# jgrodzki/radix_sort

Measured on AMD Instinct MI355X. Metric: Gkeys/sec (u64), higher is better.
Workload: dtype u64

## Files before the change

radix_sort_amd/csrc/rsx.hip:

```cpp
#include "rsx_internal.hpp"
#include "rsx_misc_kernels.hpp"
#include "rsx_any_kernels.hpp"

#include <cmath>

using namespace rsx;
using namespace rsxh;

namespace {

bool layout_ok(const rsx_layout* L, bool any_width = false) {
    if (!L) return false;
    const uint32_t kb = L->key_bytes;
    if (any_width ? (kb < 1 || kb > 16) : !(kb == 1 || kb == 2 || kb == 4 || kb == 8 || kb == 16)) return false;
    if (L->key_kind > RSX_KEY_FLOAT) return false;
    if (L->key_kind == RSX_KEY_FLOAT && !(kb == 4 || kb == 8)) return false;
    if (L->elem_bytes == 0 || (uint64_t)L->key_offset + kb > L->elem_bytes) return false;
    return true;
}
const EsLaunchers* launchers_for(uint32_t es) {
    switch (es) {
        case 1: return &es_launchers<1>();
        case 2: return &es_launchers<2>();
        case 4: return &es_launchers<4>();
// ... 247 lines not shown
                       BT, xor_mask);
    RSX_HIP(hipGetLastError());
    ctx->last_path = PATH_COUNT16;
    return RSX_OK;
}

uint32_t wide_cap(uint32_t es) { return bucket_cape((int)es, wide_kpt_for((int)es), 1024); }
bool wide_forecast(rsx_ctx* ctx, size_t n, const rsx_layout* L, hipStream_t st) {
    const uint32_t es = L->elem_bytes, D = L->key_bytes;
    const bool wide_type = es >= 8 && D >= 4;
    const size_t wide_floor = D >= 8 ? 0 : es == 8 ? ((size_t)1 << 30) : ((size_t)2 << 30);
    const bool wide_size = wide_type && (uint64_t)n > mid_max_elems((int)es);
    bool wide = false;
    if (ctx->wide_mode == 2) {
        wide = wide_type && n >= 65536;
    } else if (((ctx->wide_mode == 1 && n * (size_t)es >= wide_floor) || ctx->wide_mode == 3) && wide_size &&
               (uint64_t)n / 65536u < (uint64_t)wide_cap(es)) {
        volatile uint32_t& hint = host_word(ctx, HV_WIDE_HINT);
        const uint64_t sig = 1ull | (uint64_t)(63 - __builtin_clzll((unsigned long long)n)) << 8 | (uint64_t)es << 16 | (uint64_t)L->key_offset << 24 |
                             (uint64_t)D << 32 | (uint64_t)L->key_kind << 40;
        if (ctx->wide_skip > 0 && sig == ctx->wide_refused_sig) {
            --ctx->wide_skip;
        } else if (hint == 2u && sig == ctx->wide_tried_sig) {
            hint = 0;
            ctx->wide_skip = 15;
            ctx->wide_refused_sig = sig;
        } else {
            if (hint == 2u) hint = 0;
            wide = true;
            ctx->wide_tried_sig = sig;
        }
    }
    return wide && !((ctx->ovf16 == nullptr || ctx->wide_buf == nullptr) && capturing(st));
}
int sort_wide(rsx_ctx* ctx, const EsLaunchers& K, void* d_data, void* d_tmp, size_t n, const rsx_layout* L, hipStream_t st) {
    const uint32_t es = L->elem_bytes, D = L->key_bytes;
    int rc = ensure_ovf16(ctx, st);
    if (rc) return rc;
    if (!ctx->wide_buf) {
        RSX_HIP(hipMalloc(reinterpret_cast<void**>(&ctx->wide_buf), WIDE_BUF_BYTES));
        RSX_HIP(hipMemsetAsync(reinterpret_cast<char*>(ctx->wide_buf) + WIDE_PLAN_OFFSET, 0, sizeof(WidePlan), st));
    }
    uint64_t* tot = reinterpret_cast<uint64_t*>(ctx->wide_buf);
    uint64_t* BT = tot + 65536;
    uint64_t* starts = BT + 256;
    WidePlan* plan = reinterpret_cast<WidePlan*>(reinterpret_cast<char*>(ctx->wide_buf) + WIDE_PLAN_OFFSET);
    const uint32_t* verdict = &plan->verdict;
    const RegionGeom geom = make_geom(ctx, n, es);
    size_t parts = n * (size_t)es / (32768 * sizeof(uint32_t));
    if (parts > (size_t)ctx->num_cu) parts = (size_t)ctx->num_cu;
    static_assert(bucket_cape(8, wide_kpt_for(8), 1024) < 0x8000u && bucket_cape(4, wide_kpt_for(4), 1024) < 0x8000u, "a bucket that fits LDS must not overflow a 16-bit counter");
    uint32_t k = ctx->wide_mode == 2 ? 0u : (uint32_t)(parts / geom.num_regions);
    if (k > 0) parts = (size_t)k * geom.num_regions;
    rc = K.wideplan(ctx, d_data, n, L, plan, st);
    if (rc) return rc;
    rc = K.count16top(ctx, d_data, n, L, plan, static_cast<uint32_t*>(d_tmp), (uint32_t)parts, geom.region_shift, k, st);
    if (rc) return rc;
    {
        LaunchTimer lt(ctx, RSX_PROF_SCAN, st);
        hipLaunchKernelGGL(rsx_total16_kernel, dim3(256), dim3(256), 0, st, static_cast<const uint32_t*>(d_tmp), (uint32_t)parts, ctx->ovf16, tot, BT);
        RSX_HIP(hipGetLastError());
        const uint64_t cap1024 = wide_big_form((int)es, n) ? wide_cap(es) : bucket_cap((int)es), cap512 = bucket_cap((int)es) / 2;
        hipLaunchKernelGGL(rsx_scan16_kernel, dim3(256), dim3(256), 0, st, tot, BT, starts, cap512 / 2, cap512, cap1024, group_shift(ctx, n, L),
                           ctx->wide_mode == 2 ? 1u : 0u, (uint64_t)bucket_cape((int)es, medium_kpt_for((int)es), 1024) * 150u, (uint64_t)n / 64u, plan,
                           ctx->host_err_dev + HV_WIDE_HINT, reinterpret_cast<uint32_t*>(ctx->wide_buf + WIDE_LEFT_OFFSET));
        RSX_HIP(hipGetLastError());
    }
    SortRun lsd;
    rc = begin_control(ctx, lsd, st, geom, false);
    if (rc) return rc;
    ctx->cb_last = lsd.cb;
    SortRun hyb = lsd;
    hyb.gate = Gate{verdict, VERDICT_PATH_MASK, VERDICT_HYBRID};
    hyb.spec_dev = &plan->specs[0];
    if (k > 0) {
        rc = K.marginal16(ctx, hyb, static_cast<const uint32_t*>(d_tmp), (uint32_t)parts, k, geom, J_of(ctx, hyb, 0), J_of(ctx, hyb, 1), st);
    } else {
        rc = K.hist(ctx, hyb, d_data, geom, L, D - 2, J_of(ctx, hyb, 0), J_of(ctx, hyb, 1), true, st);
    }
    if (rc) return rc;
    rc = K.sweep(ctx, hyb, SweepPass{0, false, 0}, d_data, d_tmp, geom, L, D - 2, J_of(ctx, hyb, 0), J_of(ctx, hyb, 1), nullptr, 1, st);
    if (rc) return rc;
    hyb.spec_dev = &plan->specs[1];
    rc = K.sweep(ctx, hyb, SweepPass{1, true, 0}, d_tmp, d_data, geom, L, D - 1, J_of(ctx, hyb, 1), nullptr, nullptr, 0, st);
    if (rc) return rc;
    rc = K.bucket16(ctx, hyb, d_data, d_tmp, n, L, starts, plan, st);
    if (rc) return rc;
    lsd.gate = Gate{verdict, VERDICT_PATH_MASK, VERDICT_LSD};
    rc = lsd_passes(ctx, K, lsd, d_data, d_tmp, n, L, geom, false, 0, st);
    if (rc) return rc;
    ctx->last_sort_passes = D;
    ctx->last_path = PATH_WIDE;
    end_control(ctx);
    return RSX_OK;
}

uint32_t mid_forecast(rsx_ctx* ctx, size_t n, bool* bucket_small) {
    const uint32_t hint = host_word(ctx, HV_MID_HINT);
    uint32_t mid_mode;
    if (ctx->mid_choice == 1 && hint == 2 && ctx->mid_cooldown == 0) ctx->mid_cooldown = 8;
    if (ctx->mid_cooldown > 0) {
        --ctx->mid_cooldown;
        mid_mode = 2;
    } else {
        mid_mode = hint == 2 ? 2u : 1u;
    }
    if (ctx->mid_force) mid_mode = ctx->mid_force;
    ctx->mid_choice = mid_mode;
    *bucket_small = hint == 1 && (uint64_t)n <= 256ull * 2048ull;
    return mid_mode;
}
int sort_mid_split(rsx_ctx* ctx, const EsLaunchers& K, void* d_data, void* d_tmp, size_t n, const rsx_layout* L, bool bucket_small, hipStream_t st) {
    int rc = K.mid_split(ctx, d_data, d_tmp, n, L, st);
    if (rc) return rc;
    rc = K.bucket_sort(ctx, d_tmp, d_data, L, bucket_small, st);
    if (rc) return rc;
    ctx->last_path = PATH_MID_SPLIT;
    return RSX_OK;
}

int sort_lsd(rsx_ctx* ctx, const EsLaunchers& K, void* d_data, void* d_tmp, size_t n, const rsx_layout* L, bool mid, uint32_t mid_mode,
             hipStream_t st) {
    const RegionGeom geom = make_geom(ctx, n, L->elem_bytes);
    SortRun run;
    int rc = begin_control(ctx, run, st, geom, mid);
    if (rc) return rc;
    rc = lsd_passes(ctx, K, run, d_data, d_tmp, n, L, geom, mid, mid_mode, st);
    if (rc) return rc;
    end_control(ctx);
    return RSX_OK;
}

int sort_counting8(rsx_ctx* ctx, const EsLaunchers& K, void* d_data, size_t n, const rsx_layout* L, hipStream_t st) {
    const RegionGeom geom = make_geom(ctx, n, L->elem_bytes);
    SortRun run;
    int rc = begin_control(ctx, run, st, geom, false);
    if (rc) return rc;
    rc = K.hist(ctx, run, d_data, geom, L, 0, J_of(ctx, run, 0), nullptr, false, st);
    if (rc) return rc;
    LaunchTimer lt(ctx, RSX_PROF_OTHER, st);
    const uint64_t steps = ((n + 15) / 16 + 255) / 256;
    uint64_t blocks = steps;
    if (blocks > (uint64_t)ctx->num_cu * 16) blocks = (uint64_t)ctx->num_cu * 16;
    hipLaunchKernelGGL(rsx_expand_bytes_kernel, dim3((uint32_t)blocks), dim3(256), 0, st, static_cast<uint8_t*>(d_data),
                       (uint64_t)n, J_of(ctx, run, 0), geom.num_regions, status32(geom) ? 1u : 0u,
                       L->key_kind == RSX_KEY_SIGNED ? 0x80u : 0u);
    RSX_HIP(hipGetLastError());
    end_control(ctx);
    ctx->last_path = PATH_COUNT8;
    return RSX_OK;
}

int sort_device_locked(rsx_ctx* ctx, void* d_data, void* d_tmp, size_t n, const rsx_layout* L, hipStream_t st) {
    const EsLaunchers* K = launchers_for(L->elem_bytes);
    if (!K) return fail(ctx, RSX_ERR_UNSUPPORTED, "element size has no device kernel");
    int rc = pending_error(ctx);
    if (rc) return rc;
    rc = ensure_workspace(ctx, n, L, st);
    if (rc) return rc;
    Enqueue enq(ctx, st);
    const uint32_t D = L->key_bytes;
    const bool general_bytes = (ctx->options & OPT_GENERAL_BYTES) != 0;
    const bool counting8 = L->elem_bytes == 1 && !general_bytes;
    note_path(ctx, PATH_LSD, 0);
    if (!counting8 && n <= (size_t)512 * kpt_for((int)L->elem_bytes) && !(ctx->options & OPT_NO_SMALL_SORT)) {
        ctx->last_path = PATH_SMALL;
        return K->small_sort(ctx, d_data, n, L, st);
// ... 2427 lines not shown
```

radix_sort_amd/csrc/rsx_device.hpp:

```cpp
#pragma once
#include <hip/hip_runtime.h>
#include <stdint.h>

#include <type_traits>

namespace rsx {

constexpr int WAVE = 64;
constexpr int RADIX = 256;

template <int ES>
struct Elem;
template <>
struct Elem<1> {
    uint8_t w[1];
};
template <>
struct Elem<2> {
    uint16_t w[1];
};
template <>
struct alignas(4) Elem<4> {
    uint32_t w[1];
};
// ... 353 lines not shown
    static constexpr int SHIFT = 30;
    static constexpr uint32_t MASK = (1u << 30) - 1;
};
template <>
struct Status<uint64_t> {
    static constexpr int SHIFT = 62;
    static constexpr uint64_t MASK = (1ull << 62) - 1;
};

struct SweepArgs {
    const void* src;
    void* dst;
    RegionGeom g;
    const unsigned long long* J;
    void* status;
    uint32_t* tickets;
    const uint32_t* prev_mode;
    uint16_t wg_first[MAX_REGIONS + 1];
    void* status_clean;
    uint32_t rank_atomic;
    uint32_t hot_lanes;
    uint32_t tiles_per_region;
    uint32_t local_mask;
    unsigned long long* jnext;
    unsigned long long* jzero;
    uint32_t* error;
    DigitSpec spec;
    DigitSpec next;
    const DigitSpec* spec_dev;
    KeyXform xf;
    uint32_t opts;
    const unsigned long long* mid_J;
    DigitSpec mid_spec;
    uint32_t mid_cap;
    uint32_t mid_mode;
    uint32_t* mid_hint;
    Gate gate;
    uint32_t dbg;
    unsigned long long* dbg_cnt;
};
constexpr bool sweep_wide_cnt(int es, int kpt, int wg) { return es <= 4 && kpt >= 16 && wg <= 512; }
constexpr uint32_t SWEEP_OPT_DYNAMIC = 1u;
constexpr uint32_t SWEEP_OPT_NO_XCD_MAJOR = 2u;
constexpr uint32_t SWEEP_OPT_AGENT_STATUS = 4u;
constexpr uint32_t SWEEP_OPT_RANK_CHECK = 8u;
constexpr uint32_t SWEEP_OPT_PREREAD = 16u;
#ifdef RSX_TUNING
#define RSX_DBG(a, bit) ((a).dbg & (bit))
#else
#define RSX_DBG(a, bit) 0u
#endif

#ifdef RSX_STAMPS
#define RSX_STAMP(k)                                                   \
    do {                                                               \
        const unsigned long long _t = __builtin_amdgcn_s_memtime();    \
        stamp_acc[k] += _t - stamp_prev;                               \
        stamp_prev = _t;                                               \
    } while (0)
#else
#define RSX_STAMP(k) do {} while (0)
#endif
#ifndef RSX_MINW
#define RSX_MINW 6
#endif
#ifndef RSX_WO_PREREAD
#define RSX_WO_PREREAD 16
#endif
#ifndef RSX_START_STAGGER
#define RSX_START_STAGGER 224
#endif
#ifndef RSX_NUM_SGPR
#define RSX_NUM_SGPR 102
#endif
#ifndef RSX_RANK_GROUP
#define RSX_RANK_GROUP 4
#endif
#ifndef RSX_MINW_BIG
#define RSX_MINW_BIG 4
#endif
#ifndef RSX_WO_GROUP
#define RSX_WO_GROUP 4
#endif
#ifndef RSX_MINW_1024
#define RSX_MINW_1024 8
#endif
#ifndef RSX_ROLLCALL_TICKS
#define RSX_ROLLCALL_TICKS 40000
#endif

template <int ES, int KPT>
__device__ __forceinline__ void forget(Elem<ES> (&e)[KPT]) {
#pragma unroll
    for (int j = 0; j < KPT; ++j) {
        if constexpr (ES < 4) {
            uint32_t t = e[j].w[0];
            asm volatile("" : "+v"(t));
            e[j].w[0] = (decltype(e[j].w[0]))t;
        } else {
#pragma unroll
            for (int k = 0; k < ES / 4; ++k) asm volatile("" : "+v"(e[j].w[k]));
        }
    }
}

template <bool DPP>
__device__ __forceinline__ uint32_t wave_incl_scan(uint32_t x) {
  if constexpr (DPP) {
    auto step = [](uint32_t v, auto ctrl, auto rows) {
        return v + (uint32_t)__builtin_amdgcn_update_dpp(0, (int)v, decltype(ctrl)::value, decltype(rows)::value, 0xf, false);
    };
    x = step(x, std::integral_constant<int, 0x111>{}, std::integral_constant<int, 0xf>{});
    x = step(x, std::integral_constant<int, 0x112>{}, std::integral_constant<int, 0xf>{});
    x = step(x, std::integral_constant<int, 0x114>{}, std::integral_constant<int, 0xf>{});
    x = step(x, std::integral_constant<int, 0x118>{}, std::integral_constant<int, 0xf>{});
    x = step(x, std::integral_constant<int, 0x142>{}, std::integral_constant<int, 0xa>{});
    x = step(x, std::integral_constant<int, 0x143>{}, std::integral_constant<int, 0xc>{});
    return x;
  } else {
    const uint32_t lane = threadIdx.x & 63;
#pragma unroll
    for (int o = 1; o < 64; o <<= 1) {
        const uint32_t y = __shfl_up(x, o);
        if (lane >= (uint32_t)o) x += y;
    }
    return x;
  }
}

__device__ __forceinline__ void count_next(uint32_t* s_jn, uint32_t bin) {
    const uint32_t b0 = (uint32_t)__builtin_amdgcn_readfirstlane((int)bin);
    const uint64_t same = __ballot(bin == b0);
    if (bin == b0) {
        if (mbcnt64(same) == 0) atomicAdd(&s_jn[b0], (uint32_t)__popcll(same));
    } else {
        atomicAdd(&s_jn[bin], 1u);
    }
}

template <int ES, int KPT>
__device__ __forceinline__ void load_tile(Elem<ES> (&e)[KPT], const Elem<ES>* __restrict__ tile_ptr, uint32_t seg,
                                          uint32_t valid, bool full) {
    if (full) {
        const Elem<ES>* p0 = tile_ptr + seg;
#pragma unroll
        for (int j = 0; j < KPT; ++j) e[j] = p0[j * WAVE];
    } else {
#pragma unroll
        for (int j = 0; j < KPT; ++j) {
            const uint32_t p = seg + j * WAVE;
            if (p < valid) e[j] = tile_ptr[p];
            else e[j] = Elem<ES>{};
        }
    }
}

template <int ES, int KPT, int WG, typename S, int XF, bool NEXT, bool MID = false, bool STR = false>
__global__ __launch_bounds__(WG, (WG == 1024 ? RSX_MINW_1024 : ES == 16 ? 6 : KPT * (ES < 4 ? 4 : ES) >= 64 ? RSX_MINW_BIG : RSX_MINW))
__attribute__((amdgpu_num_sgpr(RSX_NUM_SGPR))) void rsx_sweep_kernel(const SweepArgs a) {
    constexpr int NWAVE = WG / WAVE;
    constexpr int TILE = WG * KPT;
    constexpr bool PREFETCH = ES >= 12;
    constexpr bool EARLY_HOP = ES <= 4;
    static_assert(WG >= RADIX, "need one thread per digit");
    static_assert(TILE <= 65536 / 2, "wave counters are 16 bit");
    using E = Elem<ES>;

    extern __shared__ __attribute__((aligned(16))) unsigned char smem[];
    constexpr size_t TILE_BYTES = (size_t)TILE * sizeof(E);
    E* s_elems = reinterpret_cast<E*>(smem);
    constexpr bool WIDE_CNT = sweep_wide_cnt(ES, KPT, WG);
    using Cnt = typename std::conditional<WIDE_CNT, uint32_t, uint16_t>::type;
    uint32_t* s_whist2 = reinterpret_cast<uint32_t*>(smem + TILE_BYTES);
    Cnt* s_whist = reinterpret_cast<Cnt*>(s_whist2);
    uint64_t* s_base = reinterpret_cast<uint64_t*>(s_whist2);
    uint32_t* s_jn = s_whist2 + NWAVE * RADIX * sizeof(Cnt) / 4;
    uint32_t* s_misc = s_jn + (NEXT ? a.g.num_regions * RADIX : 0);
    static_assert(NWAVE * RADIX * sizeof(Cnt) >= RADIX * sizeof(uint64_t), "s_base must fit in s_whist");

    if (!gate_open(a.gate)) return;
    const E* __restrict__ src = static_cast<const E*>(a.src);
    S* status = static_cast<S*>(a.status);
    const uint32_t NR = a.g.num_regions;
    const uint32_t tpr = a.tiles_per_region;
    const uint64_t region_len = 1ull << a.g.region_shift;

    if (NEXT)
        for (uint32_t i = threadIdx.x; i < a.g.num_regions * RADIX; i += WG) s_jn[i] = 0;
    using JT = S;
    if (a.jzero != nullptr)
        for (uint32_t i = blockIdx.x * WG + threadIdx.x; i < (uint32_t)J_REPL * NR * RADIX; i += gridDim.x * WG)
            reinterpret_cast<JT*>(a.jzero)[i] = 0;

    const uint32_t bx = (gridDim.x % 8u == 0u && !(a.opts & SWEEP_OPT_NO_XCD_MAJOR)) ? (blockIdx.x % 8u) * (gridDim.x / 8u) + blockIdx.x / 8u : blockIdx.x;
    uint32_t home = 0;
    while (home + 1 < NR && bx >= a.wg_first[home + 1]) ++home;
    const uint32_t st_step = a.wg_first[home + 1] - a.wg_first[home];
    uint32_t st_k = bx - a.wg_first[home];
    uint32_t st_nt;
    {
        const uint64_t rbeg = (uint64_t)home << a.g.region_shift;
        const uint64_t rlen = (a.g.n - rbeg) < region_len ? (a.g.n - rbeg) : region_len;
        st_nt = (uint32_t)((rlen + TILE - 1) / TILE);
    }
    E e[KPT];
    bool preloaded = false;
    uint64_t rbase = 0;
    uint64_t* s_scan = reinterpret_cast<uint64_t*>(s_misc + 16);
    uint64_t* s_half = reinterpret_cast<uint64_t*>(s_elems);
    static_assert(TILE_BYTES >= 2 * RADIX * sizeof(uint64_t), "scratch of the prefix phase lives in the tile area");
    auto load_counts = [&](const unsigned long long* Jm, uint32_t r, uint64_t& tot, uint64_t& below) {
        tot = 0;
        below = 0;
        constexpr uint32_t HALVES = WG >= 2 * RADIX ? 2 : 1;
        constexpr uint32_t RPH = J_REPL / HALVES;
        uint32_t t = threadIdx.x;
        asm volatile("" : "+v"(t));
        if (t < HALVES * RADIX) {
            const JT* col = reinterpret_cast<const JT*>(Jm) + (size_t)(t >> 8) * RPH * NR * RADIX + (t & 255u);
            constexpr uint32_t QU = ES >= 16 ? 4 : 8;
            for (uint32_t q0 = 0; q0 < NR; q0 += QU) {
#pragma unroll
                for (uint32_t qq = 0; qq < QU; ++qq) {
                    const uint32_t q = q0 + qq;
                    if (q < NR) {
#pragma unroll
                        for (uint32_t rep = 0; rep < RPH; ++rep) {
                            const uint64_t c = col[(size_t)(rep * NR + q) * RADIX];
                            tot += c;
                            below += q < r ? c : 0ull;
                        }
                    }
                }
            }
        }
    };
    auto scan_cursors = [&](uint64_t tot, uint64_t below) {
        const uint32_t t = threadIdx.x;
        if (WG >= 2 * RADIX && t >= RADIX && t < 2 * RADIX) {
            s_half[t - RADIX] = tot;
            s_half[t] = below;
        }
        __syncthreads();
        if (WG >= 2 * RADIX && t < RADIX) {
            tot += s_half[t];
            below += s_half[RADIX + t];
// ... 443 lines not shown
            }
            uint32_t spins = 0;
#ifdef RSX_STAMPS
            const unsigned long long lbs_t0 = __builtin_amdgcn_s_memtime();
            if (tid == 0 && kt > 0) ++lbs_tiles;
#endif
            while (lb_left != 0) {
#ifdef RSX_STAMPS
                if (tid == 0) ++lbs_hops;
#endif
                if (!lb_step()) {
#ifdef RSX_STAMPS
                    if (tid == 0) ++lbs_spins;
#endif
                    if (++spins > (1u << 22)) {
                        __hip_atomic_store(a.error, 1u, __ATOMIC_RELAXED, __HIP_MEMORY_SCOPE_SYSTEM);
                        break;
                    }
                    __builtin_amdgcn_s_sleep(1);
                }
            }
#ifdef RSX_STAMPS
            if (tid == 0 && kt > 0) lbs_cycles += __builtin_amdgcn_s_memtime() - lbs_t0;
#endif
            s_base[tid] = rbase + (uint64_t)lb_excl - (uint64_t)tstart;
        }
        __syncthreads();
        RSX_STAMP(5);
        if (prefetch) issue_next();

        if (!RSX_DBG(a, 2u)) {
            E* __restrict__ dst = static_cast<E*>(a.dst);
            auto next_bin = [&](uint64_t idx, const E& x) -> uint32_t {
                uint32_t r;
                if constexpr (sizeof(S) == 4)
                    r = __builtin_amdgcn_alignbit((uint32_t)(idx >> 32), (uint32_t)idx, a.g.region_shift);
                else
                    r = (uint32_t)(idx >> a.g.region_shift);
                return (r << 8) | sweep_digit<ES, STR>(x, next);
            };
            if (full) {
                auto write_full = [&](auto crowd, uint32_t hot_nd) __attribute__((always_inline)) {
                    constexpr bool CROWD = decltype(crowd)::value;
                    uint32_t hot_bin = ~0u, hot_acc = 0;
                    auto hot_flush = [&]() __attribute__((always_inline)) {
                        if (hot_acc != 0 && lane == 0) atomicAdd(&s_jn[hot_bin], hot_acc);
                        hot_acc = 0;
                    };
#pragma unroll
                    for (int i = 0; i < KPT; ++i) {
                        const uint32_t p = i * WG + tid;
                        E x;
                        if (i < PREREAD && preread) x = e[i];
                        else x = s_elems[slot_of(i)];
                        const uint64_t idx = s_base[sweep_digit<ES, STR>(x, spec)] + p;
                        if constexpr ((XF & 2) != 0) {
                            E y = x;
                            key_map<ES, true>(y, a.xf);
                            dst[idx] = y;
                        } else {
                            dst[idx] = x;
                        }
                        if constexpr (NEXT) {
                          if (!MID || do_next) {
                            if constexpr (CROWD) {
                                const uint32_t bin = next_bin(idx, x);
                                uint64_t same = __ballot(bin == hot_bin);
                                if (same == 0) {
                                    hot_flush();
                                    hot_bin = ((uint32_t)__builtin_amdgcn_readfirstlane((int)(bin >> 8)) << 8) | hot_nd;
                                    same = __ballot(bin == hot_bin);
                                    if (same == 0) {
                                        hot_bin = (uint32_t)__builtin_amdgcn_readfirstlane((int)bin);
                                        same = __ballot(bin == hot_bin);
                                    }
                                }
                                hot_acc += (uint32_t)__popcll(same);
                                if (bin != hot_bin) atomicAdd(&s_jn[bin], 1u);
                            } else if (!RSX_DBG(a, 0x8u)) {
                                atomicAdd(&s_jn[next_bin(idx, x)], 1u);
                            }
                          }
                        }
                        if (i % RSX_WO_GROUP == RSX_WO_GROUP - 1) __builtin_amdgcn_sched_barrier(0);
                    }
                    if constexpr (NEXT && CROWD) hot_flush();
                };
                bool crowded_next = false;
                uint32_t hot_nd = 0;
                if (do_next) {
                    const uint32_t nd = sweep_digit<ES, STR>(s_elems[sw0], next);
                    hot_nd = (uint32_t)__builtin_amdgcn_readfirstlane((int)nd);
                    crowded_next = __popcll(__ballot(nd == hot_nd)) >= 16;
                }
                if (crowded_next) write_full(std::true_type{}, hot_nd);
                else write_full(std::false_type{}, 0u);
            } else {
#pragma unroll
                for (int i = 0; i < KPT; ++i) {
                    const uint32_t p = i * WG + tid;
                    if (p < valid) {
                        const E x = s_elems[slot_of(i)];
                        const uint64_t idx = s_base[sweep_digit<ES, STR>(x, spec)] + p;
                        if constexpr ((XF & 2) != 0) {
                            E y = x;
                            key_map<ES, true>(y, a.xf);
                            dst[idx] = y;
                        } else {
                            dst[idx] = x;
                        }
                        if (do_next)
                            count_next(s_jn, next_bin(idx, x));
                    }
                }
            }
        }
        __syncthreads();
        RSX_STAMP(6);
    }

    if (do_next) {
        for (uint32_t i = threadIdx.x; i < a.g.num_regions * RADIX; i += WG) {
            const uint32_t c = s_jn[i];
            if (c)
                __hip_atomic_fetch_add(reinterpret_cast<JT*>(a.jnext) + (blockIdx.x % J_REPL) * (a.g.num_regions * RADIX) + i, (JT)c,
                                       __ATOMIC_RELAXED, __HIP_MEMORY_SCOPE_AGENT);
        }
    }
#ifdef RSX_STAMPS
    asm volatile("s_waitcnt vmcnt(0)" ::: "memory");
    __syncthreads();
    const unsigned long long stamp_end = __builtin_amdgcn_s_memtime();
    if ((threadIdx.x & 63) == 0)
        for (int k = 0; k < 8; ++k) atomicAdd(&a.dbg_cnt[(threadIdx.x >> 6) * 8 + k], stamp_acc[k]);
    if (threadIdx.x == 0) {
        atomicAdd(&a.dbg_cnt[64], stamp_called - stamp_entry);
        atomicAdd(&a.dbg_cnt[65], stamp_loop - stamp_called);
        atomicAdd(&a.dbg_cnt[66], stamp_end - stamp_prev);
        atomicAdd(&a.dbg_cnt[67], 1ull);
        atomicAdd(&a.dbg_cnt[68], lbs_hops);
        atomicAdd(&a.dbg_cnt[69], lbs_spins);
        atomicAdd(&a.dbg_cnt[70], lbs_cycles);
        atomicAdd(&a.dbg_cnt[71], lbs_tiles);
    }
#endif
}

template <int ES>
__global__ __launch_bounds__(256) void rsx_segcopy_kernel(const Elem<ES>* __restrict__ src,
                                                          Elem<ES>* __restrict__ dst,
                                                          const uint64_t* __restrict__ src_off,
                                                          const uint64_t* __restrict__ dst_off,
                                                          const uint64_t* __restrict__ len, uint32_t nseg,
                                                          uint32_t blocks_per_seg) {
    const uint32_t seg = blockIdx.x / blocks_per_seg;
    const uint32_t sub = blockIdx.x % blocks_per_seg;
    if (seg >= nseg) return;
    const uint64_t L = len[seg];
    const uint64_t so = src_off[seg], dof = dst_off[seg];
    for (uint64_t i = (uint64_t)sub * blockDim.x + threadIdx.x; i < L; i += (uint64_t)blocks_per_seg * blockDim.x)
        dst[dof + i] = src[so + i];
}

enum : uint32_t {
    SEGP_VALUES = 0,
    SEGP_LOCAL = 1,
// ... 5 lines not shown
```

radix_sort_amd/csrc/rsx_internal.hpp:

```cpp
#pragma once
#include "rsx_device.hpp"

#include <hip/hip_runtime.h>

#include <cstdio>
#include <cstdlib>
#include <cstring>
#include <mutex>
#include <new>
#include <algorithm>
#include <string>
#include <thread>
#include <utility>
#include <vector>

#include "../../include/rsx.h"

namespace rsxh {
using namespace rsx;

constexpr int MAX_PASSES = 16;
constexpr size_t J_BYTES = (size_t)J_REPL * MAX_REGIONS * RADIX * sizeof(uint64_t);
constexpr size_t TICKET_WORDS = ROLL_SHARDS + (size_t)ROLL_SHARD_COUNT * ROLL_SHARD_STRIDE;
constexpr uint32_t PART_MAX_SUB = 16;
// ... 143 lines not shown
        hipError_t _e = (call);                                         \
        if (_e != hipSuccess) return fail(ctx, RSX_ERR_HIP, #call, _e); \
    } while (0)

struct LaunchTimer {
    rsx_ctx* c;
    int kind;
    hipStream_t st;
    std::pair<hipEvent_t, hipEvent_t> ev{nullptr, nullptr};
    LaunchTimer(rsx_ctx* ctx, int k, hipStream_t s) : c(ctx), kind(k), st(s) {
        if (!c->prof) return;
        if (!c->prof_free.empty()) {
            ev = c->prof_free.back();
            c->prof_free.pop_back();
        } else if (hipEventCreate(&ev.first) != hipSuccess || hipEventCreate(&ev.second) != hipSuccess) {
            ev = {nullptr, nullptr};
            return;
        }
        (void)hipEventRecord(ev.first, st);
    }
    ~LaunchTimer() {
        if (!ev.first) return;
        (void)hipEventRecord(ev.second, st);
        c->prof_pending[kind].push_back(ev);
    }
};

#ifndef RSX_REGION_FLOOR
#define RSX_REGION_FLOOR 6
#endif
#ifndef RSX_KPT4
#define RSX_KPT4 28
#endif
#ifndef RSX_KPT2
#define RSX_KPT2 RSX_KPT4
#endif
#ifndef RSX_WG4
#define RSX_WG4 512
#endif
#ifndef RSX_KPT8
#define RSX_KPT8 14
#endif
#ifndef RSX_KPT16
#define RSX_KPT16 5
#endif
#ifndef RSX_KPT12
#define RSX_KPT12 10
#endif
#ifndef RSX_KPT32
#define RSX_KPT32 3
#endif
#ifndef RSX_KPT24
#define RSX_KPT24 5
#endif
#ifndef RSX_WG8
#define RSX_WG8 512
#endif
constexpr int bucket_kpt_for(int es) { return es <= 4 ? 28 : es == 8 ? 17 : es == 12 ? 9 : es == 16 ? 7 : es == 24 ? 4 : 3; }
constexpr int wide_kpt_for(int es) { return es <= 4 ? 28 : es == 8 ? 17 : es == 12 ? 12 : es == 16 ? 9 : es == 24 ? 6 : 5; }
#ifndef RSX_KMED8
#define RSX_KMED8 15
#endif
constexpr int medium_kpt_for(int es) { return es == 8 ? RSX_KMED8 : wide_kpt_for(es); }
constexpr bool wide_big_form(int es, uint64_t n) { return n / 65536u > (uint64_t)1024 * (uint64_t)bucket_kpt_for(es) * 7u / 8u; }
constexpr uint32_t LDS_PER_CU = 163840u;
constexpr size_t bucket_cnt_bytes() { return 4; }
constexpr uint32_t lds_tile_fixed(int wg) { return (uint32_t)(wg / 64) * 256u * (uint32_t)bucket_cnt_bytes() + 64u + 3u * 256u * 4u; }
constexpr uint32_t bucket_cape(int es, int kpt, int wg) {
    const uint32_t slots = (uint32_t)wg * (uint32_t)kpt;
    const uint32_t room = ((LDS_PER_CU - 1024u - lds_tile_fixed(wg)) / (uint32_t)es) & ~3u;
    return slots < room ? slots : room;
}
constexpr size_t lds_tile_bytes(int es, int kpt, int wg) { return (size_t)bucket_cape(es, kpt, wg) * (size_t)es + lds_tile_fixed(wg); }
constexpr uint32_t segment_cap(int es, int cls) { return bucket_cape(es, bucket_kpt_for(es), cls == 0 ? 256 : 1024); }
constexpr size_t WIDE_PLAN_OFFSET = (65536 + 256 + 65537 + 1) * sizeof(uint64_t);
constexpr size_t WIDE_LEFT_OFFSET = (WIDE_PLAN_OFFSET + sizeof(WidePlan) + 127) / 128 * 128;
constexpr size_t WIDE_DONE_OFFSET = WIDE_LEFT_OFFSET + 128;
constexpr size_t WIDE_BUF_BYTES = WIDE_DONE_OFFSET + 65536;
constexpr uint32_t bucket_cap(int es) { return 1024u * (uint32_t)bucket_kpt_for(es); }
constexpr uint64_t mid_max_elems(int es) { return es == 1 ? 0 : es == 8 ? (1ull << 22) : (uint64_t)bucket_cap(es) * 256u * 4u / 7u; }
constexpr int kpt_for(int es) { return es <= 2 ? RSX_KPT2 : es <= 4 ? RSX_KPT4 : es == 8 ? RSX_KPT8 : es == 12 ? RSX_KPT12 : es == 16 ? RSX_KPT16 : es == 24 ? RSX_KPT24 : RSX_KPT32; }
constexpr int wg_for(int es) { return es <= 4 ? RSX_WG4 : es == 8 ? RSX_WG8 : 512; }
constexpr uint32_t tile_elems(int es) { return wg_for(es) * kpt_for(es); }
constexpr int mid_kpt_for(int es) { return es <= 4 ? 8 : es == 8 ? 4 : es == 12 ? 3 : 2; }
constexpr uint32_t mid_tile_elems(int es) { return 512u * (uint32_t)mid_kpt_for(es); }

inline uint32_t log2u(uint64_t x) { return 63u - (uint32_t)__builtin_clzll(x); }

inline RegionGeom make_geom(const rsx_ctx* ctx, uint64_t n, uint32_t es, bool small_tiles = false) {
    RegionGeom g;
    g.n = n;
    g.tile = small_tiles ? mid_tile_elems((int)es) : tile_elems((int)es);
    uint32_t k = log2u(g.tile);
    if ((1ull << k) < g.tile) ++k;
    k += small_tiles ? 3 : RSX_REGION_FLOOR;
    const uint64_t cap = small_tiles ? MID_MAX_REGIONS : ctx->max_regions ? ctx->max_regions : (es == 8 || es == 32) ? 16 : 8;
    while (((n + (1ull << k) - 1) >> k) > cap) ++k;
    g.region_shift = k;
    g.num_regions = (uint32_t)((n + (1ull << k) - 1) >> k);
    if (g.num_regions == 0) g.num_regions = 1;
    return g;
}
inline uint64_t tiles_per_region(const RegionGeom& g) {
    return ((1ull << g.region_shift) + g.tile - 1) / g.tile;
}
inline uint64_t status_rows(const RegionGeom& g) {
    return (uint64_t)g.num_regions * tiles_per_region(g);
}
inline bool status32(const RegionGeom& g) { return g.region_shift <= 30; }

inline void ensure_lds(rsx_ctx* ctx, const void* kernel, size_t bytes) {
    for (const void* k : ctx->lds_attr)
        if (k == kernel) return;
    (void)hipFuncSetAttribute(kernel, hipFuncAttributeMaxDynamicSharedMemorySize, (int)bytes);
    ctx->lds_attr.push_back(kernel);
}

inline DigitSpec make_spec(const rsx_layout* L, uint32_t digit) {
    DigitSpec s;
    const uint32_t byte = L->key_offset + digit;
    const uint32_t top = L->key_offset + L->key_bytes - 1;
    if (L->elem_bytes >= 4) {
        s.word = byte >> 2;
        s.shift = 8 * (byte & 3);
        s.top_word = top >> 2;
        s.top_shift = 8 * (top & 3) + 7;
    } else {
        s.word = 0;
        s.shift = 8 * byte;
        s.top_word = 0;
        s.top_shift = 8 * top + 7;
    }
    s.flip = (L->key_kind != RSX_KEY_UNSIGNED && digit == L->key_bytes - 1) ? 0x80u : 0u;
    s.fsign = L->key_kind == RSX_KEY_FLOAT ? ~0u : 0u;
    return s;
}

inline char* cb_of(rsx_ctx* c, uint32_t which) { return c->aux + (size_t)which * CB_BYTES; }
inline unsigned long long* J_of(rsx_ctx* c, const SortRun& run, uint32_t which) {
    char* p = which == 0 ? cb_of(c, run.cb) + CB_J0 : which == 1 ? c->aux + OFF_J1 : c->aux + OFF_J2;
    return reinterpret_cast<unsigned long long*>(p);
}
inline unsigned long long* JT_of(rsx_ctx* c, const SortRun& run) { return reinterpret_cast<unsigned long long*>(cb_of(c, run.cb) + CB_JT); }
inline uint32_t* tickets_of(rsx_ctx* c, const SortRun& run, uint32_t pass) {
    return reinterpret_cast<uint32_t*>(cb_of(c, run.cb) + CB_TICKETS) + (size_t)pass * TICKET_WORDS;
}
inline uint32_t* part_tickets_of(rsx_ctx* c) { return reinterpret_cast<uint32_t*>(c->aux + OFF_PART_TICKETS); }
inline uint32_t* flags_of(rsx_ctx* c) { return reinterpret_cast<uint32_t*>(c->aux + OFF_FLAGS); }
inline volatile uint32_t& host_word(rsx_ctx* c, uint32_t w) { return reinterpret_cast<volatile uint32_t*>(c->host_err)[w]; }

inline uint32_t group_shift(const rsx_ctx* ctx, size_t n, const rsx_layout* L) {
    const uint64_t avg = (uint64_t)n / 65536u;
    uint32_t gs = 0;
    if (L->key_bytes >= 8 && ctx->bucket_group)
        while (gs < 6 && (avg << (gs + 1)) <= (uint64_t)512 * bucket_kpt_for((int)L->elem_bytes) * 3 / 4) ++gs;
    return gs >= 2 ? gs : 0;
}

struct SegPairsCall {
    void* keys;
    void* values;
    void* w0;
    void* w1;
    size_t n;
    uint32_t kb, vb;
    uint32_t kind, desc;
    uint32_t mode;
    uint32_t ib;
    const uint64_t* offsets;
    uint64_t nseg, row_len, max_len;
};
inline bool segment_pairs_mem(uint32_t es, const uint64_t* offsets, uint64_t row_len, uint64_t max_len) {
    const uint64_t cap = segment_cap((int)es, 1);
    return offsets ? (max_len == 0 || max_len > cap) : row_len > cap;
}

struct TopkCall {
    const void* keys;
    void* out_keys;
    void* out_index;
    void* w0;
    void* w1;
    uint64_t rows, row_len, k;
    uint32_t kb, kind, desc, ib;
};
inline uint32_t topk_max_k(uint32_t es) { return segment_cap((int)es, 1) / 2u; }
inline size_t topk_workspace_half(uint32_t es, uint64_t rows, uint64_t row_len, uint64_t k) {
    const uint64_t L = segment_cap((int)es, 1);
    if (row_len <= L) return 0;
    const uint64_t cpr = (row_len + L - 1) / L, last = row_len - (cpr - 1) * L;
// ... 157 lines not shown
```

radix_sort_amd/csrc/rsx_launch_impl.hpp:

```cpp
#pragma once
#include <cstdlib>
#include "rsx_internal.hpp"
#include "rsx_small_kernel.hpp"
#include "rsx_mid_kernels.hpp"
#include "rsx_segment_kernels.hpp"
#include "rsx_segment_pairs_kernels.hpp"
#include "rsx_topk_kernels.hpp"

#ifndef RSX_HIST_BLOCKS_PER_CU
#define RSX_HIST_BLOCKS_PER_CU 8
#endif

namespace rsxh {

inline uint32_t rank_atomic_of(const rsx_ctx* ctx) { return (ctx->rank_atomic && !(ctx->options & OPT_BALLOT_RANKS)) ? 1u : 0u; }
constexpr CleanList CLEAN_NONE = {{nullptr, nullptr, nullptr}, {0, 0, 0}};

inline uint64_t hist_blocks_per_region(const rsx_ctx* ctx, const RegionGeom& g) {
    const uint64_t per_block = 512ull * 16;
    uint64_t bpr = ((1ull << g.region_shift) + per_block - 1) / per_block;
    const uint64_t cap = ((uint64_t)ctx->num_cu * RSX_HIST_BLOCKS_PER_CU + g.num_regions - 1) / g.num_regions;
    if (bpr > cap) bpr = cap;
    return bpr == 0 ? 1 : bpr;
}
template <int ES, bool FLT>
int launch_hist_t(rsx_ctx* ctx, SortRun& run, const void* src, const RegionGeom& g, const rsx_layout* L, uint32_t digit,
                  unsigned long long* J, unsigned long long* jclear, bool clear_status, hipStream_t st) {
    const uint64_t zero16_n = clear_status ? status_rows(g) * RADIX * (status32(g) ? 4u : 8u) / 16u : 0u;
    const uint64_t bpr = hist_blocks_per_region(ctx, g);
    LaunchTimer lt(ctx, RSX_PROF_HIST, st);
    hipLaunchKernelGGL((rsx_hist_kernel<ES, FLT>), dim3((uint32_t)(bpr * g.num_regions)), dim3(512), 0, st,
                       static_cast<const Elem<ES>*>(src), g, make_spec(L, digit), (uint32_t)bpr, J, jclear, status32(g) ? 1u : 0u,
                       static_cast<uint4*>(ctx->status), zero16_n, run.clean, run.gate, DigitSpec{}, nullptr, run.spec_dev);
    RSX_HIP(hipGetLastError());
    run.clean = CLEAN_NONE;
    return RSX_OK;
}
template <int ES>
int launch_hist(rsx_ctx* ctx, SortRun& run, const void* src, const RegionGeom& g, const rsx_layout* L, uint32_t digit,
                unsigned long long* J, unsigned long long* jclear, bool clear_status, hipStream_t st) {
    if (L->key_kind == RSX_KEY_FLOAT || (L->key_kind == RSX_KEY_SIGNED && (digit + 1 == L->key_bytes || run.spec_dev != nullptr)))
        return launch_hist_t<ES, true>(ctx, run, src, g, L, digit, J, jclear, clear_status, st);
    return launch_hist_t<ES, false>(ctx, run, src, g, L, digit, J, jclear, clear_status, st);
}

template <int ES>
int launch_hist2(rsx_ctx* ctx, SortRun& run, const void* src, const RegionGeom& g, const rsx_layout* L, uint32_t digit,
                 unsigned long long* J, uint32_t digit2, unsigned long long* J2, unsigned long long* jclear, hipStream_t st) {
    const uint64_t zero16_n = status_rows(g) * RADIX * (status32(g) ? 4u : 8u) / 16u;
    const uint64_t bpr = hist_blocks_per_region(ctx, g);
    LaunchTimer lt(ctx, RSX_PROF_HIST, st);
    if (L->key_kind != RSX_KEY_UNSIGNED)
        hipLaunchKernelGGL((rsx_hist_kernel<ES, true, true>), dim3((uint32_t)(bpr * g.num_regions)), dim3(512), 0, st,
                           static_cast<const Elem<ES>*>(src), g, make_spec(L, digit), (uint32_t)bpr, J, jclear, status32(g) ? 1u : 0u,
                           static_cast<uint4*>(ctx->status), zero16_n, run.clean, run.gate, make_spec(L, digit2), J2);
    else
        hipLaunchKernelGGL((rsx_hist_kernel<ES, false, true>), dim3((uint32_t)(bpr * g.num_regions)), dim3(512), 0, st,
                           static_cast<const Elem<ES>*>(src), g, make_spec(L, digit), (uint32_t)bpr, J, jclear, status32(g) ? 1u : 0u,
                           static_cast<uint4*>(ctx->status), zero16_n, run.clean, run.gate, make_spec(L, digit2), J2);
    RSX_HIP(hipGetLastError());
    run.clean = CLEAN_NONE;
    return RSX_OK;
}

inline KeyXform make_xform(const rsx_layout* L) {
    KeyXform x;
    std::memset(&x, 0, sizeof x);
    if (L->key_kind == RSX_KEY_UNSIGNED) return x;
    const uint32_t top = L->key_offset + L->key_bytes - 1;
    auto word_of = [&](uint32_t byte) { return L->elem_bytes >= 4 ? byte >> 2 : 0u; };
    auto bit_of = [&](uint32_t byte) { return L->elem_bytes >= 4 ? 8 * (byte & 3) : 8 * byte; };
    const uint32_t sw = word_of(top);
    const uint32_t sbit = 1u << (bit_of(top) + 7);
    x.sign[sw] = sbit;
    x.xpos[sw] = sbit;
    if (L->key_kind == RSX_KEY_SIGNED) {
        x.xneg[sw] = sbit;
    } else {
        for (uint32_t b = L->key_offset; b <= top; ++b) x.xneg[word_of(b)] |= 0xFFu << bit_of(b);
    }
    return x;
}

template <int ES, typename S, int XF, bool NEXT, bool MID = false, bool STR = false>
int launch_sweep_t(rsx_ctx* ctx, const SortRun& run, const SweepPass& pass, const void* src, void* dst, const RegionGeom& g, const rsx_layout* L,
                   uint32_t digit, const unsigned long long* J, unsigned long long* jnext, unsigned long long* jzero,
                   hipStream_t st) {
    constexpr int KPT = kpt_for(ES);
    if (g.tile != (uint32_t)(wg_for(ES) * KPT)) return fail(ctx, RSX_ERR_INTERNAL, "launch_sweep: geometry of another tile size");
    constexpr int SWEEP_WG = wg_for(ES);
    constexpr int TILE = SWEEP_WG * KPT;
    char* const half[2] = {static_cast<char*>(ctx->status), static_cast<char*>(ctx->status) + ctx->status_bytes};
    const uint32_t which = pass.index & 1u;
    SweepArgs a;
    a.status_clean = pass.last ? nullptr : half[which ^ 1u];
    a.src = src;
    a.dst = dst;
    a.g = g;
    a.J = J;
    a.status = half[which];
    a.tickets = run.tickets_override ? run.tickets_override : tickets_of(ctx, run, pass.index);
    a.prev_mode = pass.index ? tickets_of(ctx, run, pass.index - 1) + ROLL_SHARDS + 1 : nullptr;
    a.jnext = jnext;
    a.jzero = jzero;
    a.error = ctx->host_err_dev;
    a.spec = make_spec(L, digit);
    a.next = make_spec(L, NEXT ? digit + 1 : digit);
    a.spec.flip = a.next.flip = 0;
    a.xf = make_xform(L);
    a.tiles_per_region = (uint32_t)tiles_per_region(g);
    a.opts = ((ctx->options & OPT_DYNAMIC_TILES) ? SWEEP_OPT_DYNAMIC : 0u) |
             ((ctx->options & OPT_NO_XCD_MAJOR) ? SWEEP_OPT_NO_XCD_MAJOR : 0u) |
             ((ctx->options & OPT_AGENT_STATUS) || !ctx->l2_local ? SWEEP_OPT_AGENT_STATUS : 0u) |
             ((ctx->options & OPT_RANK_CHECK) ? SWEEP_OPT_RANK_CHECK : 0u) |
             ((uint64_t)g.n * ES <= (2ull << 30) ? SWEEP_OPT_PREREAD : 0u);
    a.dbg = ctx->dbg;
    a.mid_J = nullptr;
    a.mid_spec = a.spec;
    a.mid_cap = 0;
    a.gate = run.gate;
    a.spec_dev = run.spec_dev;
    a.mid_mode = pass.mid;
    a.mid_hint = ctx->host_err_dev + HV_MID_HINT;
    if constexpr (MID) {
        a.mid_J = JT_of(ctx, run);
        a.mid_spec = make_spec(L, L->key_bytes - 1);
        a.mid_spec.flip = 0;
        a.mid_cap = bucket_cap(ES);
    }
    a.rank_atomic = rank_atomic_of(ctx);
    a.hot_lanes = (ctx->options & OPT_ATOMIC_RANKS) ? 65u : ctx->hot_lanes;
    a.dbg_cnt = reinterpret_cast<unsigned long long*>(ctx->aux + OFF_DBG);
    const size_t lds = (size_t)TILE * ES + (SWEEP_WG / WAVE) * RADIX * (sweep_wide_cnt(ES, KPT, SWEEP_WG) ? sizeof(uint32_t) : sizeof(uint16_t)) +
                       (NEXT ? (size_t)g.num_regions * RADIX * sizeof(uint32_t) : 0) + 128;
    auto kern = rsx_sweep_kernel<ES, KPT, SWEEP_WG, S, XF, NEXT, MID, STR>;
    thread_local size_t occ_lds = ~(size_t)0;
    thread_local int occ = 0;
    if (occ == 0 || occ_lds != lds) {
        int o = 0;
        if (hipOccupancyMaxActiveBlocksPerMultiprocessor(&o, kern, SWEEP_WG, lds) != hipSuccess || o < 1) o = 2;
        occ = o;
        occ_lds = lds;
    }
    const uint32_t NR = g.num_regions;
    const uint64_t region_len = 1ull << g.region_shift;
    auto tiles_of = [&](uint32_t r) -> uint64_t {
        const uint64_t beg = (uint64_t)r << g.region_shift;
        const uint64_t len = g.n - beg < region_len ? g.n - beg : region_len;
        return (len + TILE - 1) / TILE;
    };
    uint64_t real_tiles = 0;
    for (uint32_t r = 0; r < NR; ++r) real_tiles += tiles_of(r);
    uint64_t grid = (uint64_t)ctx->num_cu * occ;
    if (grid > real_tiles) grid = real_tiles;
    if (grid < NR) grid = NR;
#ifdef RSX_TUNING
    if (const char* o = std::getenv("RSX_OCC")) {
        const long v = std::atol(o);
        if (v >= 1 && v <= 8) grid = (uint64_t)ctx->num_cu * (uint64_t)v;
    }
#endif
    if (grid > 0xFFFFu) grid = 0xFFFFu;
    {
        uint64_t cum = 0;
        for (uint32_t r = 0; r < NR; ++r) {
            a.wg_first[r] = (uint16_t)(cum * grid / real_tiles);
            cum += tiles_of(r);
        }
        a.wg_first[NR] = (uint16_t)grid;
        for (uint32_t r = 0; r < NR; ++r)
            if (a.wg_first[r + 1] <= a.wg_first[r]) a.wg_first[r + 1] = a.wg_first[r] + 1;
        for (uint32_t r = NR; r-- > 0;) {
            const uint32_t cap = (uint32_t)grid - (NR - r);
            if (a.wg_first[r] > cap) a.wg_first[r] = (uint16_t)cap;
        }
        a.wg_first[NR] = (uint16_t)grid;
        for (uint32_t r = NR + 1; r <= (uint32_t)MAX_REGIONS; ++r) a.wg_first[r] = (uint16_t)grid;
        a.local_mask = 0;
        if (grid % 8 == 0 && !(ctx->options & OPT_NO_XCD_MAJOR))
            for (uint32_t r = 0; r < NR; ++r)
                if (a.wg_first[r] / (grid / 8) == (a.wg_first[r + 1] - 1u) / (grid / 8)) a.local_mask |= 1u << r;
    }
    if (ctx->options & OPT_VERBOSE) std::fprintf(stderr, "[rsx] sweep ES=%d NEXT=%d occ=%d grid=%llu lds=%zu tiles=%llu regions=%u\n", ES, (int)NEXT, occ, (unsigned long long)grid, lds, (unsigned long long)real_tiles, g.num_regions);
    LaunchTimer lt(ctx, RSX_PROF_SWEEP, st);
    hipLaunchKernelGGL(kern, dim3((uint32_t)grid), dim3(SWEEP_WG), lds, st, a);
    RSX_HIP(hipGetLastError());
    return RSX_OK;
}

template <int ES, typename S, int XF>
int launch_sweep_n(rsx_ctx* ctx, const SortRun& run, const SweepPass& pass, const void* src, void* dst, const RegionGeom& g, const rsx_layout* L,
                   uint32_t digit, const unsigned long long* J, unsigned long long* jnext, unsigned long long* jzero,
                   hipStream_t st) {
    if (run.spec_dev != nullptr) {
        if constexpr (ES >= 8 && (XF & 2) == 0) {
            if (jnext) return launch_sweep_t<ES, S, XF, true, false, true>(ctx, run, pass, src, dst, g, L, digit, J, jnext, jzero, st);
            if constexpr (XF == 0) return launch_sweep_t<ES, S, 0, false, false, true>(ctx, run, pass, src, dst, g, L, digit, J, nullptr, jzero, st);
        }
        return fail(ctx, RSX_ERR_INTERNAL, "launch_sweep: no kernel for this pass of the hybrid");
    }
    if constexpr ((XF & 2) == 0) {
        if constexpr (sizeof(S) == 4 && ES != 1) {
            if (jnext && pass.mid != 0) return launch_sweep_t<ES, S, XF, true, true>(ctx, run, pass, src, dst, g, L, digit, J, jnext, jzero, st);
        }
        if (jnext) return launch_sweep_t<ES, S, XF, true>(ctx, run, pass, src, dst, g, L, digit, J, jnext, jzero, st);
    } else if (jnext) {
        return fail(ctx, RSX_ERR_ARG, "a last pass cannot count for a next one");
    }
    return launch_sweep_t<ES, S, XF, false>(ctx, run, pass, src, dst, g, L, digit, J, nullptr, jzero, st);
}

template <int ES, typename S>
int launch_sweep_x(rsx_ctx* ctx, const SortRun& run, const SweepPass& pass, const void* src, void* dst, const RegionGeom& g, const rsx_layout* L,
                   uint32_t digit, const unsigned long long* J, unsigned long long* jnext, unsigned long long* jzero,
                   int xf, hipStream_t st) {
    switch (L->key_kind == RSX_KEY_UNSIGNED ? 0 : xf) {
        case 1: return launch_sweep_n<ES, S, 1>(ctx, run, pass, src, dst, g, L, digit, J, jnext, jzero, st);
        case 2: return launch_sweep_n<ES, S, 2>(ctx, run, pass, src, dst, g, L, digit, J, jnext, jzero, st);
        case 3: return launch_sweep_n<ES, S, 3>(ctx, run, pass, src, dst, g, L, digit, J, jnext, jzero, st);
        default: return launch_sweep_n<ES, S, 0>(ctx, run, pass, src, dst, g, L, digit, J, jnext, jzero, st);
    }
}

template <int ES>
int launch_sweep(rsx_ctx* ctx, const SortRun& run, const SweepPass& pass, const void* src, void* dst, const RegionGeom& g, const rsx_layout* L,
                 uint32_t digit, const unsigned long long* J, unsigned long long* jnext, unsigned long long* jzero, int xf, hipStream_t st) {
    if (status32(g)) return launch_sweep_x<ES, uint32_t>(ctx, run, pass, src, dst, g, L, digit, J, jnext, jzero, xf, st);
    return launch_sweep_x<ES, uint64_t>(ctx, run, pass, src, dst, g, L, digit, J, jnext, jzero, xf, st);
}

inline SmallArgs small_args(const rsx_ctx* ctx, const rsx_layout* L, uint32_t passes, uint32_t nspec, bool map_load) {
    SmallArgs a;
    std::memset(&a, 0, sizeof a);
    a.passes = passes;
    a.rank_atomic = rank_atomic_of(ctx);
    a.map_store = L->key_kind == RSX_KEY_UNSIGNED ? 0u : 1u;
    a.map_load = map_load ? a.map_store : 0u;
    for (uint32_t d = 0; d < nspec; ++d) {
        a.spec[d] = make_spec(L, d);
        a.spec[d].flip = 0;
    }
    a.xf = make_xform(L);
    a.no_skip = ctx->bucket_no_skip;
    a.key_offset = L->key_offset;
    a.key_bytes = L->key_bytes;
    return a;
}

template <int ES>
int launch_small_sort(rsx_ctx* ctx, void* data, size_t n, const rsx_layout* L, hipStream_t st) {
    constexpr int KPT = kpt_for(ES);
    if (n == 0 || n > (size_t)512 * KPT || L->key_bytes > 16) return fail(ctx, RSX_ERR_INTERNAL, "launch_small_sort: size out of range");
    SmallArgs a = small_args(ctx, L, L->key_bytes, L->key_bytes, true);
    a.src = data;
    a.data = data;
    a.n = (uint32_t)n;
    const size_t lds = (size_t)512 * KPT * ES + 8 * RADIX * sizeof(uint32_t) + 64;
    auto kern = rsx_small_sort_kernel<ES, KPT>;
    LaunchTimer lt(ctx, RSX_PROF_OTHER, st);
    hipLaunchKernelGGL(kern, dim3(1), dim3(512), lds, st, a);
    RSX_HIP(hipGetLastError());
    return RSX_OK;
}

inline uint32_t* mid_totals_of(rsx_ctx* ctx) { return reinterpret_cast<uint32_t*>(ctx->aux + OFF_BASE); }
template <int ES>
int launch_mid_split(rsx_ctx* ctx, const void* src, void* dst, size_t n, const rsx_layout* L, hipStream_t st) {
    if constexpr (ES == 1) {
        return fail(ctx, RSX_ERR_INTERNAL, "launch_mid_split: one-byte elements");
    } else {
        constexpr int KPT = mid_kpt_for(ES);
        constexpr uint32_t TILE = 512u * KPT;
        MidArgs a;
        std::memset(&a, 0, sizeof a);
        a.src = src;
        a.dst = dst;
        a.n = (uint32_t)n;
        a.tiles = (uint32_t)((n + TILE - 1) / TILE);
        if ((size_t)a.tiles * RADIX * sizeof(uint32_t) > ctx->status_bytes) return fail(ctx, RSX_ERR_INTERNAL, "launch_mid_split: workspace");
        a.C = static_cast<uint32_t*>(ctx->status);
// ... 370 lines not shown
```

Measured before the change: 81.24.

## Use a deeper tile and store throttling for the hybrid's final wide sweep

For 8-byte keys, the hybrid path's second sweep (which counts nothing for a next pass) now runs with a larger keys-per-thread tile, using its own region geometry. A guard checks that its status rows fit inside those the first sweep zeroes. The kernel for that variant also inserts a vmcnt wait after each write-out group, capping outstanding stores. The aim is to amortize per-tile lookback and scatter overhead and to smooth write traffic, at the cost of more LDS per workgroup and possible stalls from the store throttle.

```diff
diff --git a/radix_sort_amd/csrc/rsx.hip b/radix_sort_amd/csrc/rsx.hip
--- a/radix_sort_amd/csrc/rsx.hip
+++ b/radix_sort_amd/csrc/rsx.hip
@@ -353,7 +353,10 @@
     rc = K.sweep(ctx, hyb, SweepPass{0, false, 0}, d_data, d_tmp, geom, L, D - 2, J_of(ctx, hyb, 0), J_of(ctx, hyb, 1), nullptr, 1, st);
     if (rc) return rc;
     hyb.spec_dev = &plan->specs[1];
-    rc = K.sweep(ctx, hyb, SweepPass{1, true, 0}, d_tmp, d_data, geom, L, D - 1, J_of(ctx, hyb, 1), nullptr, nullptr, 0, st);
+    const RegionGeom geom2 = ctx->wide_mode == 2 ? geom : hyb_geom(geom, es);
+    if (status_rows_used(geom2) > status_rows_used(geom) || tiles_per_region(geom2) > tiles_per_region(geom))
+        return fail(ctx, RSX_ERR_INTERNAL, "sort_wide: the second sweep's status rows are not among those the first one zeroes");
+    rc = K.sweep(ctx, hyb, SweepPass{1, true, 0}, d_tmp, d_data, geom2, L, D - 1, J_of(ctx, hyb, 1), nullptr, nullptr, 0, st);
     if (rc) return rc;
     rc = K.bucket16(ctx, hyb, d_data, d_tmp, n, L, starts, plan, st);
     if (rc) return rc;
diff --git a/radix_sort_amd/csrc/rsx_device.hpp b/radix_sort_amd/csrc/rsx_device.hpp
--- a/radix_sort_amd/csrc/rsx_device.hpp
+++ b/radix_sort_amd/csrc/rsx_device.hpp
@@ -459,6 +459,9 @@
 #ifndef RSX_WO_GROUP
 #define RSX_WO_GROUP 4
 #endif
+#ifndef RSX_WO_STORES
+#define RSX_WO_STORES 3
+#endif
 #ifndef RSX_MINW_1024
 #define RSX_MINW_1024 8
 #endif
@@ -539,6 +542,7 @@
     constexpr int TILE = WG * KPT;
     constexpr bool PREFETCH = ES >= 12;
     constexpr bool EARLY_HOP = ES <= 4;
+    constexpr bool WO_THROTTLE = ES == 8 && STR && !MID && !PREFETCH;
     static_assert(WG >= RADIX, "need one thread per digit");
     static_assert(TILE <= 65536 / 2, "wave counters are 16 bit");
     using E = Elem<ES>;
@@ -1148,6 +1152,7 @@
                             }
                           }
                         }
+                        if constexpr (WO_THROTTLE) asm volatile("s_waitcnt vmcnt(%0)" ::"n"(RSX_WO_STORES) : "memory");
                         if (i % RSX_WO_GROUP == RSX_WO_GROUP - 1) __builtin_amdgcn_sched_barrier(0);
                     }
                     if constexpr (NEXT && CROWD) hot_flush();
diff --git a/radix_sort_amd/csrc/rsx_internal.hpp b/radix_sort_amd/csrc/rsx_internal.hpp
--- a/radix_sort_amd/csrc/rsx_internal.hpp
+++ b/radix_sort_amd/csrc/rsx_internal.hpp
@@ -249,6 +249,11 @@
 constexpr int kpt_for(int es) { return es <= 2 ? RSX_KPT2 : es <= 4 ? RSX_KPT4 : es == 8 ? RSX_KPT8 : es == 12 ? RSX_KPT12 : es == 16 ? RSX_KPT16 : es == 24 ? RSX_KPT24 : RSX_KPT32; }
 constexpr int wg_for(int es) { return es <= 4 ? RSX_WG4 : es == 8 ? RSX_WG8 : 512; }
 constexpr uint32_t tile_elems(int es) { return wg_for(es) * kpt_for(es); }
+#ifndef RSX_HYB_KPT8
+#define RSX_HYB_KPT8 18
+#endif
+constexpr int hyb_kpt_for(int es) { return es == 8 ? RSX_HYB_KPT8 : kpt_for(es); }
+static_assert((size_t)RSX_WG8 * RSX_HYB_KPT8 * 8 + (RSX_WG8 / 64) * 256 * 2 + 128 <= LDS_PER_CU / 2, "the deep tile leaves no room for two workgroups per CU");
 constexpr int mid_kpt_for(int es) { return es <= 4 ? 8 : es == 8 ? 4 : es == 12 ? 3 : 2; }
 constexpr uint32_t mid_tile_elems(int es) { return 512u * (uint32_t)mid_kpt_for(es); }
 
@@ -273,6 +278,15 @@
 }
 inline uint64_t status_rows(const RegionGeom& g) {
     return (uint64_t)g.num_regions * tiles_per_region(g);
+}
+inline RegionGeom hyb_geom(const RegionGeom& g, uint32_t es) {
+    RegionGeom d = g;
+    d.tile = (uint32_t)wg_for((int)es) * (uint32_t)hyb_kpt_for((int)es);
+    return d;
+}
+inline uint64_t status_rows_used(const RegionGeom& g) {
+    const uint64_t last = g.n - ((uint64_t)(g.num_regions - 1) << g.region_shift);
+    return (uint64_t)(g.num_regions - 1) * tiles_per_region(g) + (last + g.tile - 1) / g.tile;
 }
 inline bool status32(const RegionGeom& g) { return g.region_shift <= 30; }
 
diff --git a/radix_sort_amd/csrc/rsx_launch_impl.hpp b/radix_sort_amd/csrc/rsx_launch_impl.hpp
--- a/radix_sort_amd/csrc/rsx_launch_impl.hpp
+++ b/radix_sort_amd/csrc/rsx_launch_impl.hpp
@@ -82,11 +82,11 @@
     return x;
 }
 
-template <int ES, typename S, int XF, bool NEXT, bool MID = false, bool STR = false>
+template <int ES, typename S, int XF, bool NEXT, bool MID = false, bool STR = false, int KPT = kpt_for(ES)>
 int launch_sweep_t(rsx_ctx* ctx, const SortRun& run, const SweepPass& pass, const void* src, void* dst, const RegionGeom& g, const rsx_layout* L,
                    uint32_t digit, const unsigned long long* J, unsigned long long* jnext, unsigned long long* jzero,
                    hipStream_t st) {
-    constexpr int KPT = kpt_for(ES);
+    static_assert(KPT == kpt_for(ES) || (STR && !NEXT && !MID), "only the hybrid's sweep that counts nothing has room for a deeper tile");
     if (g.tile != (uint32_t)(wg_for(ES) * KPT)) return fail(ctx, RSX_ERR_INTERNAL, "launch_sweep: geometry of another tile size");
     constexpr int SWEEP_WG = wg_for(ES);
     constexpr int TILE = SWEEP_WG * KPT;
@@ -195,7 +195,13 @@
     if (run.spec_dev != nullptr) {
         if constexpr (ES >= 8 && (XF & 2) == 0) {
             if (jnext) return launch_sweep_t<ES, S, XF, true, false, true>(ctx, run, pass, src, dst, g, L, digit, J, jnext, jzero, st);
-            if constexpr (XF == 0) return launch_sweep_t<ES, S, 0, false, false, true>(ctx, run, pass, src, dst, g, L, digit, J, nullptr, jzero, st);
+            if constexpr (XF == 0) {
+                if constexpr (hyb_kpt_for(ES) != kpt_for(ES)) {
+                    if (g.tile == (uint32_t)(wg_for(ES) * hyb_kpt_for(ES)))
+                        return launch_sweep_t<ES, S, 0, false, false, true, hyb_kpt_for(ES)>(ctx, run, pass, src, dst, g, L, digit, J, nullptr, jzero, st);
+                }
+                return launch_sweep_t<ES, S, 0, false, false, true>(ctx, run, pass, src, dst, g, L, digit, J, nullptr, jzero, st);
+            }
         }
         return fail(ctx, RSX_ERR_INTERNAL, "launch_sweep: no kernel for this pass of the hybrid");
     }
```

Result: faster. 83.24, median of 6 (+2.5%).
